# prophesier/diff-svc

Hardware: NVIDIA B200
Metric: audio-sec/s (1/RTF), 1000-step DDPM @44.1kHz + NSF-HiFiGAN (higher is better)
Workload: dtype f32 (fp16 hi/lo split x3 on tcgen05, fp32 accumulate)

## Files before the change

diffsvc_b200/csrc/diffnet.cu:

```cuda
#include "common.cuh"
#include "epilogues.cuh"
#include "simt_gemm.cuh"
#include "tc_pair.cuh"
#include "tc_splitk.cuh"
#include "tc_layer.cuh"
#include "tc_step.cuh"

#include <cmath>
#include <memory>

namespace dsvc {


__global__ void transpose_kernel(const float* __restrict__ in, float* __restrict__ out, Plane pl, int R, int Cc) {
  __shared__ float tile[32][33];
  const int b = blockIdx.z;
  const int c0 = blockIdx.x * 32, r0 = blockIdx.y * 32;
  const float* ib = in + (size_t)b * R * Cc;
  for (int i = threadIdx.y; i < 32; i += blockDim.y) {
    const int r = r0 + i, c = c0 + threadIdx.x;
    tile[i][threadIdx.x] = (r < R && c < Cc) ? ib[(size_t)r * Cc + c] : 0.f;
  }
  __syncthreads();
  for (int i = threadIdx.y; i < 32; i += blockDim.y) {
// ... 114 lines not shown
  int passes = 3;
  DevBuf w_in, b_in, w_dil, w_cond, b_cond, w_out, b_out, w_skip, b_skip, w_head, b_head;
  DevBuf dtab;
  F16Pair h_in, h_skip, h_head;
  std::vector<std::unique_ptr<F16Pair>> h_dil, h_out;
  DevBuf c_recip, c_recipm1, c_coef1, c_coef2, c_logvar, c_acp;
  bool have_schedule = false;
  int B = 0, Tmax = 0;
  int uB = 0, uT = 0;
  DevBuf rowmap;
  bool packed = false;
  bool prepared = false;
  DevBuf X, S, XS, hist, CP, cond_cl, lengths, state;
  PlaneBuf Y, Z, SP, R, XIN;
  PlaneBuf Y2;
  bool pingpong = false;
  int fused_usable = 0;
  TcMaps maps;
  DevBuf tile_tab;
  int tile_slots = 0, tile_live = 0;
  DevBuf step_flags;
  int step_bn = 0;
  int step_pairs = 0;
  DevBuf sk_slab;
  int num_sms = 148;
  cudaGraphExec_t g_ddpm = nullptr, g_plms = nullptr;
  cudaGraphExec_t g_ddpm_x = nullptr;
  uint64_t g_ddpm_x_nodes = 0;
  cudaStream_t cap_stream = nullptr;
  uint64_t g_ddpm_nodes = 0, g_plms_nodes = 0;
// ... 84 lines not shown
  DSVC_TRY(w0.upload(w->mlp0_w, (size_t)4 * C * C * 4, s));
  DSVC_TRY(b0.upload(w->mlp0_b, (size_t)4 * C * 4, s));
  DSVC_TRY(w2.upload(w->mlp2_w, (size_t)4 * C * C * 4, s));
  DSVC_TRY(b2.upload(w->mlp2_b, (size_t)C * 4, s));
  DSVC_TRY(upload_f(wp, wpv, s));
  DSVC_TRY(upload_f(bp, bpv, s));
  DSVC_TRY(t1.reserve((size_t)Tn * 4 * C * 4));
  DSVC_TRY(t2.reserve((size_t)Tn * C * 4));
  DSVC_TRY(h->dtab.reserve((size_t)Tn * L * C * 4));
  DSVC_TRY(gemm_affine(basis.as<float>(), w0.as<float>(), b0.as<float>(), t1.as<float>(), Tn, C, 4 * C, EpiAffine::ACT_MISH, s));
  DSVC_TRY(gemm_affine(t1.as<float>(), w2.as<float>(), b2.as<float>(), t2.as<float>(), Tn, 4 * C, C, EpiAffine::ACT_NONE, s));
  DSVC_TRY(gemm_affine(t2.as<float>(), wp.as<float>(), bp.as<float>(), h->dtab.as<float>(), Tn, C, L * C, EpiAffine::ACT_NONE, s));
  DSVC_CUDA(cudaStreamSynchronize(s));
  return DSVC_OK;
}

static int tc_build_maps(dsvc_diffnet* h) {
  const int M = h->cfg.mel_bins, C = h->cfg.residual_channels, L = h->cfg.residual_layers;
  const int B = h->B, T = h->Tmax;
  auto gemm = [&](TcGemmMaps& g, const PlaneBuf& a, int K, const F16Pair& w, int rows) -> int {
    DSVC_TRY(tc_make_a_map(&g.a_hi, a.hi.as<__half>(), B, T, K));
    DSVC_TRY(tc_make_a_map(&g.a_lo, a.lo.as<__half>(), B, T, K));
    DSVC_TRY(tc_make_b_map(&g.b_hi, w.hi.as<__half>(), rows, K, 128));
    DSVC_TRY(tc_make_b_map(&g.b_lo, w.lo.as<__half>(), rows, K, 128));
    DSVC_TRY(tc_make_b_map(&g.b32_hi, w.hi.as<__half>(), rows, K, 32));
    DSVC_TRY(tc_make_b_map(&g.b32_lo, w.lo.as<__half>(), rows, K, 32));
    DSVC_TRY(tc_make_b_map(&g.b64_hi, w.hi.as<__half>(), rows, K, 64));
    DSVC_TRY(tc_make_b_map(&g.b64_lo, w.lo.as<__half>(), rows, K, 64));
    return DSVC_OK;
  };
  DSVC_TRY(gemm(h->maps.in, h->XIN, M, h->h_in, C));
  DSVC_TRY(gemm(h->maps.skip, h->SP, C, h->h_skip, C));
  DSVC_TRY(gemm(h->maps.head, h->R, C, h->h_head, M));
  h->maps.dil.resize(L);
  h->maps.out.resize(L);
  for (int l = 0; l < L; ++l) {
    const PlaneBuf& yin = (h->pingpong && (l & 1)) ? h->Y2 : h->Y;
    DSVC_TRY(gemm(h->maps.dil[l], yin, C, *h->h_dil[l], 3 * 2 * C));
    DSVC_TRY(gemm(h->maps.out[l], h->Z, C, *h->h_out[l], 2 * C));
  }
  return DSVC_OK;
}

struct HeadArgs {
  int mode = HEAD_EVAL;
  float* out = nullptr;
  int tsel = 0;
};

static ConvGemmParams base_params(const float* A, const float* W, int B, int T, int Cin, int Cout, int taps, int dil) {
  ConvGemmParams p{};
  p.A = A; p.W = W; p.B = B; p.Lin = T; p.Cin = Cin; p.Cout = Cout; p.taps = taps; p.rows = T;
  p.in_stride = 1; p.in_off = (taps == 3) ? -dil : 0; p.tap_step = dil; p.nphase = 1; p.tpad = 0; p.in_slope = 1.0f;
  p.a_batch_stride = (long long)T * Cin;
// ... 6 lines not shown
  if (ctas128 >= 2 * 148) return launch_conv_gemm_tile<128, 128, 8, 8, Epi>(p, e, s);
  return launch_conv_gemm_tile<64, 128, 4, 8, Epi>(p, e, s);
}

static EpiInProj::Params mk_inproj(const dsvc_diffnet* h, int tsel) {
  EpiInProj::Params e{};
  e.bias = h->b_in.as<float>(); e.dtab = h->dtab.as<float>(); e.st = h->state.as<StepState>(); e.lengths = h->lengths.as<int>();
  e.X = h->X.as<float>(); e.Y = h->Y.view(h->tc); e.Tmax = h->Tmax; e.C = h->cfg.residual_channels; e.L = h->cfg.residual_layers;
  e.tsel = tsel; e.wscale = h->tc ? h->h_in.inv_scale : 1.f;
  e.rowmap = h->packed ? h->rowmap.as<int2>() : nullptr;
  return e;
}
static EpiGate::Params mk_gate(const dsvc_diffnet* h, int l) {
  const int C = h->cfg.residual_channels;
  EpiGate::Params e{};
  e.CP = h->CP.as<float>() + (size_t)l * h->B * h->Tmax * 2 * C; e.Z = h->Z.view(h->tc); e.Tmax = h->Tmax; e.C = C;
  e.fast = h->tc ? 1 : 0; e.wscale = h->tc ? h->h_dil[l]->inv_scale : 1.f;
  return e;
}
static EpiOutProj::Params mk_outproj(const dsvc_diffnet* h, int l, int tsel) {
  const int C = h->cfg.residual_channels;
  EpiOutProj::Params e{};
  e.bias = h->b_out.as<float>() + (size_t)l * 2 * C; e.dtab = h->dtab.as<float>(); e.st = h->state.as<StepState>();
  e.lengths = h->lengths.as<int>(); e.X = h->X.as<float>(); e.S = h->S.as<float>(); e.SP = h->SP.view(h->tc);
  e.Y = ((h->pingpong && ((l + 1) & 1)) ? h->Y2 : h->Y).view(h->tc);
  e.Tmax = h->Tmax; e.C = C; e.L = h->cfg.residual_layers; e.layer = l; e.tsel = tsel; e.fast = h->tc ? 1 : 0;
  e.wscale = h->tc ? h->h_out[l]->inv_scale : 1.f;
  e.rowmap = h->packed ? h->rowmap.as<int2>() : nullptr;
  return e;
}
static EpiSkipProj::Params mk_skip(const dsvc_diffnet* h) {
// ... 2 lines not shown
  e.wscale = h->tc ? h->h_skip.inv_scale : 1.f;
  return e;
}
static EpiHead::Params mk_head(const dsvc_diffnet* h, const HeadArgs& ha) {
  EpiHead::Params e{};
  e.bias = h->b_head.as<float>(); e.st = h->state.as<StepState>(); e.mode = ha.mode; e.B = h->B; e.Tmax = h->Tmax;
  e.M = h->cfg.mel_bins; e.out = ha.out; e.xs = h->XS.as<float>(); e.XIN = h->XIN.view(h->tc);
  e.c_recip = h->c_recip.as<float>(); e.c_recipm1 = h->c_recipm1.as<float>(); e.c_coef1 = h->c_coef1.as<float>();
  e.c_coef2 = h->c_coef2.as<float>(); e.c_logvar = h->c_logvar.as<float>();
  e.alphas_cumprod = h->c_acp.as<float>(); e.hist = h->hist.as<float>();
  e.wscale = h->tc ? h->h_head.inv_scale : 1.f;
  e.rowmap = h->packed ? h->rowmap.as<int2>() : nullptr; e.uB = h->uB; e.uT = h->uT;
  return e;
}

static int enqueue_layer_conv(dsvc_diffnet* h, int l, cudaStream_t s) {
  const int C = h->cfg.residual_channels, B = h->B, T = h->Tmax;
  const int dil = 1 << (l % h->cfg.dilation_cycle_length);
  const EpiGate::Params e = mk_gate(h, l);
  if (h->tc) {
    const TcGemmMaps& m = h->maps.dil[l];
    const char* skv = getenv("DSVC_SPLITK");
    const bool sk_wanted = (skv && atoi(skv) >= 1) || !tc_pair_enabled();
    if (h->passes == 3 && sk_wanted && h->tile_slots == 0 && h->sk_slab.bytes >= tc_splitk_slab_bytes(B, T, 2 * C) &&
        tc_splitk_eligible(B, T, 2 * C, 3, h->num_sms))
      return tc_splitk_launch<EpiGate>(m, e, h->sk_slab.as<float>(), B, T, C, 2 * C, dil, s);
    return tc_launch<EpiGate>(m, e, B, T, C, 2 * C, 3, dil, h->passes, s, tiles_of(h));
  }
  const float* W = h->w_dil.as<float>() + (size_t)l * 3 * 2 * C * C;
  return launch_fp32<EpiGate>(h, base_params(h->Y.f32.as<float>(), W, B, T, C, 2 * C, 3, dil), e, s);
}

static int enqueue_layer_out(dsvc_diffnet* h, int l, int tsel, cudaStream_t s) {
  const int C = h->cfg.residual_channels, B = h->B, T = h->Tmax;
  const EpiOutProj::Params e = mk_outproj(h, l, tsel);
  if (h->tc) return tc_launch<EpiOutProj>(h->maps.out[l], e, B, T, C, 2 * C, 1, 0, h->passes, s, tiles_of(h));
  const float* W = h->w_out.as<float>() + (size_t)l * 2 * C * C;
  return launch_fp32<EpiOutProj>(h, base_params(h->Z.f32.as<float>(), W, B, T, C, 2 * C, 1, 0), e, s);
}

static int enqueue_layer_fused(dsvc_diffnet* h, int l, int tsel, cudaStream_t s) {
  const int dil = 1 << (l % h->cfg.dilation_cycle_length);
  const TcGemmMaps* next = l + 1 < h->cfg.residual_layers ? &h->maps.dil[l + 1] : nullptr;
  return tc_layer_launch(h->maps.dil[l], h->maps.out[l], next, mk_gate(h, l), mk_outproj(h, l, tsel), h->B, h->Tmax,
                         h->cfg.residual_channels, dil, h->passes, s);
}

static bool fused_layers(const dsvc_diffnet* h) {
  if (h->tile_slots > 0) return false;
  if (!(h->tc && h->pingpong && h->fused_usable >= 1 &&
        tc_layer_shape_ok(h->B, h->Tmax, h->cfg.residual_channels))) return false;
  return tc_layer_env() >= 2 || (long long)ceil_div(h->Tmax, TC_BM) * h->B <= h->fused_usable;
}
// ... 57 lines not shown
  const char* sb = getenv("DSVC_STEP_BN");
  const int want = sb ? atoi(sb) : 0;
  if (want != 128 && M % 64 == 0 && C % 64 == 0 && cap64 > 0 && (n_ft * (2 * C / 64) <= cap64 || want == 64)) {
    const int S = n_ft * (2 * C / 64), R = ceil_div(S, cap64);
    h->step_pairs = ceil_div(S, R);
    return 64;
  }
  if (M % 128 == 0 && C % 128 == 0 && cap128 > 0) {
    const int S = n_ft * (2 * C / 128), R = ceil_div(S, cap128);
    h->step_pairs = ceil_div(S, R);
    return 128;
  }
  return 0;
}

static int enqueue_eval(dsvc_diffnet* h, const HeadArgs& ha, cudaStream_t s) {
  const int M = h->cfg.mel_bins, C = h->cfg.residual_channels, L = h->cfg.residual_layers;
  const int B = h->B, T = h->Tmax;
  if (h->step_bn > 0) return enqueue_eval_step(h, ha, s);
  {
    const EpiInProj::Params e = mk_inproj(h, ha.tsel);
    if (h->tc) DSVC_TRY(tc_launch<EpiInProj>(h->maps.in, e, B, T, M, C, 1, 0, h->passes, s, tiles_of(h)));
    else DSVC_TRY(launch_fp32<EpiInProj>(h, base_params(h->XIN.f32.as<float>(), h->w_in.as<float>(), B, T, M, C, 1, 0), e, s));
  }
  for (int l = 0; l < L; ++l) {
    if (fused_layers(h)) {
      DSVC_TRY(enqueue_layer_fused(h, l, ha.tsel, s));
      continue;
    }
    DSVC_TRY(enqueue_layer_conv(h, l, s));
    DSVC_TRY(enqueue_layer_out(h, l, ha.tsel, s));
  }
  {
    const EpiSkipProj::Params e = mk_skip(h);
    if (h->tc) DSVC_TRY(tc_launch<EpiSkipProj>(h->maps.skip, e, B, T, C, C, 1, 0, h->passes, s, tiles_of(h)));
    else DSVC_TRY(launch_fp32<EpiSkipProj>(h, base_params(h->SP.f32.as<float>(), h->w_skip.as<float>(), B, T, C, C, 1, 0), e, s));
  }
  {
    const EpiHead::Params e = mk_head(h, ha);
    if (h->tc) DSVC_TRY(tc_launch<EpiHead>(h->maps.head, e, B, T, C, M, 1, 0, h->passes, s, tiles_of(h)));
    else DSVC_TRY(launch_fp32<EpiHead>(h, base_params(h->R.f32.as<float>(), h->w_head.as<float>(), B, T, C, M, 1, 0), e, s));
  }
  return DSVC_OK;
}

static int load_x(dsvc_diffnet* h, const float* spec, cudaStream_t s) {
  const int M = h->cfg.mel_bins;
// ... 153 lines not shown
  }
  const bool ragged = tc && (int)tab.size() < dense;
  const bool ragged_changed = ragged != (h->tile_slots > 0);
  if (ragged) {
    h->tile_live = (int)tab.size();
    h->tile_slots = 2 * ceil_div(dense, 2);
    tab.resize(h->tile_slots, make_int2(0, -1));
    DSVC_TRY(h->tile_tab.reserve(tab.size() * sizeof(int2)));
    DSVC_CUDA(cudaMemcpyAsync(h->tile_tab.p, tab.data(), tab.size() * sizeof(int2), cudaMemcpyHostToDevice, s));
    DSVC_CUDA(cudaMemsetAsync(h->Y.hi.p, 0, n * C * sizeof(__half), s));
    DSVC_CUDA(cudaMemsetAsync(h->Y.lo.p, 0, n * C * sizeof(__half), s));
  } else {
    h->tile_slots = h->tile_live = 0;
  }
  DSVC_CUDA(cudaStreamSynchronize(s));
  if (resized || !h->prepared || ragged_changed) {
    h->g_ddpm_valid = h->g_plms_valid = false;
    if (tc) DSVC_TRY(tc_build_maps(h));
  }
  {
    const int bn = step_pick_bn(h);
    if (bn != h->step_bn) h->g_ddpm_valid = h->g_plms_valid = false;
    h->step_bn = bn;
    if (bn > 0) {
      const size_t fb = ((size_t)2 * ceil_div(Tmax, 2 * TC_BM) * 32 + 32) * sizeof(unsigned);
      DSVC_TRY(h->step_flags.reserve(fb));
      DSVC_CUDA(cudaMemsetAsync(h->step_flags.p, 0, fb, s));
    }
  }
  {
    Plane none{nullptr, nullptr, nullptr};
    dim3 grid(ceil_div(Tmax, 32), ceil_div(H, 32), B), block(32, 8);
    if (pack) pack_rows_kernel<<<grid, block, 0, s>>>(cond, h->cond_cl.as<float>(), none, h->rowmap.as<int2>(), Tmax, H, user_T);
    else
    transpose_kernel<<<grid, block, 0, s>>>(cond, h->cond_cl.as<float>(), none, H, Tmax);
    DSVC_LAUNCH_CHECK();
    ConvGemmParams p = base_params(h->cond_cl.as<float>(), h->w_cond.as<float>(), B, Tmax, H, L * 2 * C, 1, 0);
    EpiCondProj::Params e{};
    e.bias = h->b_cond.as<float>(); e.CP = h->CP.as<float>(); e.B = B; e.Tmax = Tmax; e.C2 = 2 * C;
    DSVC_TRY((launch_conv_gemm_tile<128, 128, 8, 8, EpiCondProj>(p, e, s)));
  }
  h->prepared = true;
  return DSVC_OK;
// ... 17 lines not shown
  DSVC_REQUIRE(hubert && mel2ph && f0 && pitch_embed && decoder_inp && f0_denorm, "dsvc_cond_encode: null argument");
  DSVC_REQUIRE(B > 0 && Th > 0 && T > 0 && H > 0 && f0_bin > 2, "dsvc_cond_encode: bad dimensions");
  DSVC_TRY(require_device());
  const float mel_min = (float)(1127.0 * std::log(1.0 + (double)f0_min / 700.0));
  const float mel_max = (float)(1127.0 * std::log(1.0 + (double)f0_max / 700.0));
  cond_encode_kernel<<<dim3(T, B), 128, 0, (cudaStream_t)stream>>>(hubert, reinterpret_cast<const long long*>(mel2ph), f0,
                                                                 pitch_embed, Th, T, H, f0_bin, mel_min, mel_max,
                                                                 decoder_inp, f0_denorm);
  DSVC_LAUNCH_CHECK();
  return DSVC_OK;
}

int dsvc_diffnet_run_layer(dsvc_diffnet_t* h, int32_t layer, int32_t part, int32_t iters, void* stream) {
  DSVC_REQUIRE(h, "dsvc_diffnet_run_layer: null handle");
  if (!h->prepared) { set_error("dsvc_diffnet_run_layer: call dsvc_diffnet_prepare first"); return DSVC_ESTATE; }
  DSVC_REQUIRE(layer >= 0 && layer < h->cfg.residual_layers && part >= 0 && part <= 3 && iters >= 0, "bad layer/part/iters");
  if (part == 3) {
    if (h->step_bn == 0) { set_error("dsvc_diffnet_run_layer: part 3 needs the step kernel (tc_step.cuh) for this shape"); return DSVC_ESTATE; }
    cudaStream_t s3 = (cudaStream_t)stream;
    set_state_kernel<<<1, 1, 0, s3>>>(h->state.as<StepState>(), 500, 1, 1ull, nullptr);
    DSVC_LAUNCH_CHECK();
    HeadArgs ha3; ha3.mode = HEAD_DDPM;
    for (int i = 0; i < iters; ++i) DSVC_TRY(enqueue_eval(h, ha3, s3));
#ifdef DSVC_TIMELINE
    {
      static long long tl[160][2 * STEP_MAXL + 3][10];
      DSVC_CUDA(cudaStreamSynchronize(s3));
      DSVC_CUDA(cudaMemcpyFromSymbol(tl, g_step_tl, sizeof(tl)));
      const int np = 2 * h->cfg.residual_layers + 3;
      const int nct = 2 * h->step_pairs;
      printf("step kernel timeline (last launch), cycles.  per phase of CTA c: start->deps | deps->first operands | first->MMAs issued | "
// ... 14 lines not shown
        double a[8] = {0, 0, 0, 0, 0, 0, 0, 0}; int n = 0;
        for (int c = 0; c < nct && c < 160; c += 2)
          for (int ph = 1 + par; ph < np - 2; ph += 2) {
            const long long* t = tl[c][ph];
            a[0] += t[1] - t[0]; a[1] += t[2] - t[1]; a[2] += t[3] - t[2]; a[3] += t[4] - t[3]; a[4] += t[5] - t[4]; a[5] += t[6] - t[5];
            a[6] += t[7] - t[6]; a[7] += tl[c][ph + 1][0] - t[0]; ++n;
          }
        printf("  mean %s: deps %.0f | first operands %.0f | MMA issue %.0f | acc ready %.0f | staged %.0f | epi %.0f | signal %.0f | total %.0f\n",
               par ? "out-proj" : "conv    ", a[0] / n, a[1] / n, a[2] / n, a[3] / n, a[4] / n, a[5] / n, a[6] / n, a[7] / n);
      }
      fflush(stdout);
    }
#endif
    return DSVC_OK;
  }
  if (part == 2 && !fused_layers(h)) {
    set_error("dsvc_diffnet_run_layer: part 2 (fused layer kernel) needs DSVC_FUSED_LAYER and a tensor-core handle whose "
              "2C/64 channel tiles form a schedulable cluster");
    return DSVC_ESTATE;
  }
  cudaStream_t s = (cudaStream_t)stream;
  set_state_kernel<<<1, 1, 0, s>>>(h->state.as<StepState>(), 0, 1, 0ull, nullptr);
  DSVC_LAUNCH_CHECK();
  for (int i = 0; i < iters; ++i) {
    if (part == 0) DSVC_TRY(enqueue_layer_conv(h, layer, s));
    else if (part == 1) DSVC_TRY(enqueue_layer_out(h, layer, 0, s));
    else DSVC_TRY(enqueue_layer_fused(h, layer, 0, s));
  }
#ifdef DSVC_TIMELINE
  if (h->tc) {
    static long long host_tl[1024][16];
    DSVC_CUDA(cudaStreamSynchronize(s));
    DSVC_CUDA(cudaMemcpyFromSymbol(host_tl, g_timeline, sizeof(host_tl)));
    const int nct = 2 * ceil_div(ceil_div(h->Tmax, TC_BM), 2) * ceil_div(2 * h->cfg.residual_channels, 64) * h->B;
    if (part == 2) {
      printf("timeline fused layer (cycles since CTA entry): setup | A:first-operands | A:mma-issued | A:epi-prefetch | A:acc-ready | "
             "A:staged | A:epi-done | fences | cluster-barrier | B:first-operands | B:mma-issued | B:epi-prefetch | B:acc-ready | "
             "B:staged | B:epi-done\n");
      for (int c = 0; c < nct && c < 1024; c += (nct > 12 ? nct / 12 : 1))
        printf("  cta %3d: %6lld %6lld %6lld %6lld %6lld %6lld %6lld %6lld %6lld %6lld %6lld %6lld %6lld %6lld %6lld\n", c,
// ... 93 lines not shown
```

diffsvc_b200/csrc/tc_gemm.cuh:

```cuda
#pragma once
#include <cuda.h>
#include <stdlib.h>
#include <cmath>

#include "common.cuh"
#include "epilogues.cuh"

namespace dsvc {

struct TcGemmMaps {
  CUtensorMap a_hi, a_lo;
  CUtensorMap b_hi, b_lo;
  CUtensorMap b32_hi, b32_lo;
  CUtensorMap b64_hi, b64_lo;
};
struct TcMaps {
  TcGemmMaps in, skip, head;
  std::vector<TcGemmMaps> dil, out;
};

struct TcTiles {
  const int2* tab = nullptr;
  int slots = 0, live = 0;
};
// ... 188 lines not shown
  asm volatile("tcgen05.ld.sync.aligned.32x32b.x4.b32 {%0, %1, %2, %3}, [%4];"
               : "=r"(u[0]), "=r"(u[1]), "=r"(u[2]), "=r"(u[3]) : "r"(taddr) : "memory");
  asm volatile("tcgen05.wait::ld.sync.aligned;" ::: "memory");
}
template <int CW> __device__ __forceinline__ void tmem_ld_cols(uint32_t taddr, float (&r)[CW]);
template <> __device__ __forceinline__ void tmem_ld_cols<8>(uint32_t taddr, float (&r)[8]) { tmem_ld8(taddr, r); }
template <> __device__ __forceinline__ void tmem_ld_cols<4>(uint32_t taddr, float (&r)[4]) { tmem_ld4(taddr, r); }
template <> __device__ __forceinline__ void tmem_ld_cols<32>(uint32_t taddr, float (&r)[32]) { tmem_ld32(taddr, r); }
template <> __device__ __forceinline__ void tmem_ld_cols<16>(uint32_t taddr, float (&r)[16]) { tmem_ld16(taddr, r); }

#ifdef DSVC_TIMELINE
__device__ long long g_timeline[1024][16];
#define TL_MARK(slot) do { if (lane == 0) g_timeline[((blockIdx.z * gridDim.y + blockIdx.y) * gridDim.x + blockIdx.x) & 1023][slot] = clock64() - tl0; } while (0)
#define TL_ENTRY() do { if (threadIdx.x == 0) { unsigned long long gt_; asm volatile("mov.u64 %0, %%globaltimer;" : "=l"(gt_)); \
  g_timeline[((blockIdx.z * gridDim.y + blockIdx.y) * gridDim.x + blockIdx.x) & 1023][15] = (long long)gt_; } } while (0)
#else
#define TL_MARK(slot) do { } while (0)
#define TL_ENTRY() do { } while (0)
#endif

template <class Epi, int BN, bool LEAN = false>
__device__ __forceinline__ void tc_epilogue(const typename Epi::Params& ep, uint8_t* smem_raw, uint32_t smem_base,
                                            uint32_t tmem_base, uint32_t tmem_full_bar, uint32_t tmem_parity, int T, int N,
                                            int m0, int ny, int b, int warp, int lane, bool two_acc
#ifdef DSVC_TIMELINE
                                            , long long tl0, int tl_off = 0
#endif
                                            , int pair_h = 0
                                            , uint32_t acc_free_bar = 0
) {
#ifndef DSVC_TIMELINE
    constexpr int tl_off = 0;
    (void)tl_off;
// ... 421 lines not shown
```

diffsvc_b200/csrc/tc_pair.cuh:

```cuda
#pragma once
#include "tc_gemm.cuh"

namespace dsvc {

template <int BN> struct TcPairCfg {
  static constexpr int H = BN / 2;
  static constexpr int P_TILE = BN * TC_BK * 2;
  static constexpr int STAGE = 2 * TC_A_TILE + P_TILE;
  static constexpr int STAGES = (BN == 64) ? 5 : (BN == 128 ? 4 : 3);
  static constexpr int SMEM = STAGES * STAGE + 1024  + 256 ;
  static_assert(4 * 32 * (BN + 4) * 4 <= STAGES * STAGE, "epilogue staging must fit in the operand ring");
};

__device__ __forceinline__ uint32_t mapa_cluster(uint32_t local_addr, uint32_t cta_rank) {
  uint32_t r;
  asm volatile("mapa.shared::cluster.u32 %0, %1, %2;" : "=r"(r) : "r"(local_addr), "r"(cta_rank));
  return r;
}
__device__ __forceinline__ void tma2_load_2d(const CUtensorMap* map, uint32_t bar, uint32_t dst, int c0, int c1) {
  asm volatile(
      "cp.async.bulk.tensor.2d.cta_group::2.shared::cluster.global.mbarrier::complete_tx::bytes [%0], [%1, {%3, %4}], [%2];"
      ::"r"(dst), "l"(map), "r"(bar), "r"(c0), "r"(c1) : "memory");
}
__device__ __forceinline__ void tma2_load_3d(const CUtensorMap* map, uint32_t bar, uint32_t dst, int c0, int c1, int c2) {
// ... 1 lines not shown
      "cp.async.bulk.tensor.3d.cta_group::2.shared::cluster.global.mbarrier::complete_tx::bytes [%0], [%1, {%3, %4, %5}], [%2];"
      ::"r"(dst), "l"(map), "r"(bar), "r"(c0), "r"(c1), "r"(c2) : "memory");
}
__device__ __forceinline__ void umma2_f16(uint32_t tmem_d, uint64_t adesc, uint64_t bdesc, uint32_t idesc, uint32_t accumulate) {
  asm volatile(
      "{\n\t.reg .pred p;\n\tsetp.ne.b32 p, %4, 0;\n\t"
      "tcgen05.mma.cta_group::2.kind::f16 [%0], %1, %2, %3, p;\n\t}"
      ::"r"(tmem_d), "l"(adesc), "l"(bdesc), "r"(idesc), "r"(accumulate) : "memory");
}
__device__ __forceinline__ void umma2_commit_both(uint32_t bar) {
  asm volatile("tcgen05.commit.cta_group::2.mbarrier::arrive::one.shared::cluster.multicast::cluster.b64 [%0], %1;"
               ::"r"(bar), "h"((uint16_t)3) : "memory");
}

template <class Epi, int BN>
__global__ void __launch_bounds__(TC_THREADS, 1)
tc_pair_kernel(const __grid_constant__ CUtensorMap tmAh, const __grid_constant__ CUtensorMap tmAl,
               const __grid_constant__ CUtensorMap tmBh, const __grid_constant__ CUtensorMap tmBl,
               const typename Epi::Params ep, int T, int K, int N, int taps, int dil, const int2* __restrict__ tiles) {
#if defined(__CUDA_ARCH__) && (__CUDA_ARCH__ >= 1000)
  using Cfg = TcPairCfg<BN>;
  constexpr int STAGES = Cfg::STAGES;
  constexpr int H = Cfg::H;
  pdl_launch_dependents();
  int m0 = blockIdx.x * TC_BM, b = blockIdx.z;
  if (tiles != nullptr) {
    const int2 t = __ldg(tiles + blockIdx.x), tp = __ldg(tiles + (blockIdx.x ^ 1u));
    if (t.y < 0 && tp.y < 0) return;
    b = t.y < 0 ? tp.x : t.x;
    m0 = t.y < 0 ? ((T + TC_BM - 1) / TC_BM) * TC_BM : t.y;
  }
  extern __shared__ uint8_t smem_raw[];
  const uint32_t smem_base = (smem_u32(smem_raw) + 1023u) & ~1023u;
  const uint32_t bar_base = smem_base + STAGES * Cfg::STAGE;
  auto full_bar = [&](int s) { return bar_base + 8u * s; };
// ... 33 lines not shown
  tc_fence_before();
  __syncthreads();
  cluster_sync_all();
  tc_fence_after();
  uint32_t tmem_base;
  asm volatile("ld.shared.u32 %0, [%1];" : "=r"(tmem_base) : "r"(tmem_slot) : "memory");
  if (warp == 3) TL_MARK(0);

  auto full_bar_leader = [&](int s) { return mapa_cluster(full_bar(s), 0u); };

  auto load_p = [&](int it, int s) {
    const int tap = it / kblocks, kb = it - tap * kblocks;
    if constexpr (BN == 256) {
      int r0, r1;
      if constexpr (Epi::kPair) {
        const int sb = tap * N + (int)blockIdx.y * 256;
        r0 = sb + (rank == 0 ? 0 : 64); r1 = r0 + 128;
      } else {
        r0 = tap * N + (int)blockIdx.y * 256 + (int)rank * 128; r1 = r0 + 64;
      }
      const uint32_t bar = full_bar_leader(s);
      const uint32_t p = tile_p(s);
      tma2_load_2d(&tmBh, bar, p, kb * TC_BK, r0);
      tma2_load_2d(&tmBh, bar, p + 64u * 128u, kb * TC_BK, r1);
      tma2_load_2d(&tmBl, bar, p + 128u * 128u, kb * TC_BK, r0);
      tma2_load_2d(&tmBl, bar, p + 192u * 128u, kb * TC_BK, r1);
    } else {
    int ra, rb;
    if constexpr (Epi::kPair) {
      const int per = 128 / BN;
      ra = tap * N + (int)(blockIdx.y / per) * 128 + (int)(blockIdx.y % per) * H;
      rb = ra + 64;
    } else {
      ra = tap * N + (int)blockIdx.y * BN;
      rb = ra + H;
    }
    const uint32_t bar = full_bar_leader(s);
    const uint32_t p = tile_p(s);
    tma2_load_2d(&tmBh, bar, p, kb * TC_BK, rank == 0 ? ra : rb);
    tma2_load_2d(&tmBl, bar, p + (uint32_t)H * 128u, kb * TC_BK, rank == 0 ? rb : ra);
    }
  };
  auto load_a = [&](int it, int s) {
    const int tap = it / kblocks, kb = it - tap * kblocks;
    const int frame = m0 + (tap - (taps >> 1)) * dil;
    const uint32_t bar = full_bar_leader(s);
    tma2_load_3d(&tmAh, bar, tile_a(s, 0), kb * TC_BK, frame, b);
    tma2_load_3d(&tmAl, bar, tile_a(s, 1), kb * TC_BK, frame, b);
  };

  if (warp == 0) {
    constexpr uint32_t tx_pair = 2u * Cfg::STAGE;
    const int pre = total < STAGES ? total : STAGES;
    if (elect_one_sync()) {
      for (int it = 0; it < pre; ++it) {
        if (rank == 0) mbar_expect_tx(full_bar(it), tx_pair);
        load_p(it, it);
      }
    }
    __syncwarp();
    pdl_wait();
    if (elect_one_sync()) {
      for (int it = 0; it < pre; ++it) load_a(it, it);
    }
    __syncwarp();
    for (int it = pre; it < total; ++it) {
      const int s = it % STAGES;
      const uint32_t ph = (uint32_t)(it / STAGES) & 1u;
      mbar_wait(empty_bar(s), ph ^ 1u);
      if (elect_one_sync()) {
        if (rank == 0) mbar_expect_tx(full_bar(s), tx_pair);
        load_a(it, s);
        load_p(it, s);
      }
      __syncwarp();
    }
// ... 20 lines not shown
            umma2_f16(tmem_base, al + koff, pd + koff, idesc_lo, 1u);
          } else {
            umma2_f16(tmem_base, ah + koff, pd + koff, idesc_hi, acc);
            umma2_f16(tmem_base, al + koff, pd + koff, idesc_lo, 1u);
          }
        }
        umma2_commit_both(empty_bar(s));
        if (it == total - 1) umma2_commit_both(tmem_full_bar);
      }
      __syncwarp();
    }
    TL_MARK(2);
  }
  pdl_wait();
#ifdef DSVC_TIMELINE
  tc_epilogue<Epi, BN>(ep, smem_raw, smem_base, tmem_base, tmem_full_bar, 0u, T, N, m0, (int)blockIdx.y, b, warp, lane, true, tl0, 0, BN == 256 ? 0 : H);
#else
  tc_epilogue<Epi, BN>(ep, smem_raw, smem_base, tmem_base, tmem_full_bar, 0u, T, N, m0, (int)blockIdx.y, b, warp, lane, true, BN == 256 ? 0 : H);
#endif
  if (warp == 4) TL_MARK(6);
  tc_fence_before();
  __syncthreads();
  cluster_sync_all();
  if (warp == 2) {
    tc_fence_after();
    asm volatile("tcgen05.dealloc.cta_group::2.sync.aligned.b32 %0, %1;" ::"r"(tmem_base), "n"(2 * BN) : "memory");
  }
#endif
}

inline bool tc_pair_enabled() {
  const char* e = getenv("DSVC_TC_PAIR");
  return !(e && atoi(e) == 0);
}

template <class Epi, int BN>
int tc_pair_launch_bn(const TcGemmMaps& m, const typename Epi::Params& e, int B, int T, int K, int N, int taps, int dil,
                      cudaStream_t s, TcTiles tt = TcTiles{}) {
  DSVC_TRY((ensure_dyn_smem<tc_pair_kernel<Epi, BN>>(TcPairCfg<BN>::SMEM)));
  cudaLaunchConfig_t cfg{};
  cfg.gridDim = tt.tab ? dim3(tt.slots, N / BN, 1) : dim3(2 * ceil_div(ceil_div(T, TC_BM), 2), N / BN, B);
  cfg.blockDim = dim3(TC_THREADS);
  cfg.dynamicSmemBytes = TcPairCfg<BN>::SMEM;
  cfg.stream = s;
  cudaLaunchAttribute attr[2];
  attr[0].id = cudaLaunchAttributeClusterDimension;
  attr[0].val.clusterDim.x = 2;
  attr[0].val.clusterDim.y = 1;
  attr[0].val.clusterDim.z = 1;
  attr[1].id = cudaLaunchAttributeProgrammaticStreamSerialization;
  attr[1].val.programmaticStreamSerializationAllowed = 1;
  cfg.attrs = attr;
  cfg.numAttrs = 2;
  const CUtensorMap& bh = (BN == 64) ? m.b32_hi : m.b64_hi;
  const CUtensorMap& bl = (BN == 64) ? m.b32_lo : m.b64_lo;
  DSVC_CUDA(cudaLaunchKernelEx(&cfg, tc_pair_kernel<Epi, BN>, m.a_hi, m.a_lo, bh, bl, e, T, K, N, taps, dil, tt.tab));
  DSVC_LAUNCH_CHECK();
  return DSVC_OK;
}

template <class Epi>
int tc_launch(const TcGemmMaps& m, const typename Epi::Params& e, int B, int T, int K, int N, int taps, int dil, int passes,
              cudaStream_t s, TcTiles tt = TcTiles{}) {
  DSVC_REQUIRE(K % TC_BK == 0, "tc_launch: K=%d must be a multiple of %d", K, TC_BK);
  if (passes == 3 && tc_pair_enabled()) {
    const int bn = tc_pick_bn(B, T, N, tt.live);
    if (bn == 64 && N % 64 == 0) return tc_pair_launch_bn<Epi, 64>(m, e, B, T, K, N, taps, dil, s, tt);
    if (bn == 128 && N % 128 == 0) return tc_pair_launch_bn<Epi, 128>(m, e, B, T, K, N, taps, dil, s, tt);
    if (bn == 256 && N % 256 == 0) return tc_pair_launch_bn<Epi, 256>(m, e, B, T, K, N, taps, dil, s, tt);
  }
  return tc_launch_single<Epi>(m, e, B, T, K, N, taps, dil, passes, s, tt);
// ... 4 lines not shown
```

Baseline: 29.87.

## Defer skip-half of out-projection into next layer's dilated-conv launch

Splits each layer's out-projection GEMM into a residual half (launched immediately) and a skip half, then runs that skip half as extra CTAs inside the next layer's dilated-conv kernel through a new two-role tc_pair2 kernel. Z is double-buffered (Z2) so the deferred skip CTAs still read the previous layer's gate output. The goal is to fill idle SMs when the grid is small and to take the skip accumulation off the critical path between layers. It is enabled only when the combined CTA count fits on the SMs. It adds a Z2 buffer, one extra launch for the last layer, and timeline instrumentation.

```diff
diff --git a/diffsvc_b200/csrc/diffnet.cu b/diffsvc_b200/csrc/diffnet.cu
--- a/diffsvc_b200/csrc/diffnet.cu
+++ b/diffsvc_b200/csrc/diffnet.cu
@@ -6,6 +6,8 @@
 #include "tc_layer.cuh"
 #include "tc_step.cuh"
 
+#include <algorithm>
+#include <climits>
 #include <cmath>
 #include <memory>
 
@@ -152,6 +154,8 @@
   DevBuf X, S, XS, hist, CP, cond_cl, lengths, state;
   PlaneBuf Y, Z, SP, R, XIN;
   PlaneBuf Y2;
+  PlaneBuf Z2;
+  bool skip_defer = false;
   bool pingpong = false;
   int fused_usable = 0;
   TcMaps maps;
@@ -266,6 +270,8 @@
   DSVC_CUDA(cudaStreamSynchronize(s));
   return DSVC_OK;
 }
+
+static const PlaneBuf& zplane(const dsvc_diffnet* h, int l) { return (h->skip_defer && (l & 1)) ? h->Z2 : h->Z; }
 
 static int tc_build_maps(dsvc_diffnet* h) {
   const int M = h->cfg.mel_bins, C = h->cfg.residual_channels, L = h->cfg.residual_layers;
@@ -289,7 +295,7 @@
   for (int l = 0; l < L; ++l) {
     const PlaneBuf& yin = (h->pingpong && (l & 1)) ? h->Y2 : h->Y;
     DSVC_TRY(gemm(h->maps.dil[l], yin, C, *h->h_dil[l], 3 * 2 * C));
-    DSVC_TRY(gemm(h->maps.out[l], h->Z, C, *h->h_out[l], 2 * C));
+    DSVC_TRY(gemm(h->maps.out[l], zplane(h, l), C, *h->h_out[l], 2 * C));
   }
   return DSVC_OK;
 }
@@ -326,7 +332,7 @@
 static EpiGate::Params mk_gate(const dsvc_diffnet* h, int l) {
   const int C = h->cfg.residual_channels;
   EpiGate::Params e{};
-  e.CP = h->CP.as<float>() + (size_t)l * h->B * h->Tmax * 2 * C; e.Z = h->Z.view(h->tc); e.Tmax = h->Tmax; e.C = C;
+  e.CP = h->CP.as<float>() + (size_t)l * h->B * h->Tmax * 2 * C; e.Z = zplane(h, l).view(h->tc); e.Tmax = h->Tmax; e.C = C;
   e.fast = h->tc ? 1 : 0; e.wscale = h->tc ? h->h_dil[l]->inv_scale : 1.f;
   return e;
 }
@@ -359,12 +365,22 @@
   return e;
 }
 
-static int enqueue_layer_conv(dsvc_diffnet* h, int l, cudaStream_t s) {
+static int enqueue_inproj(dsvc_diffnet* h, int tsel, cudaStream_t s) {
+  const int M = h->cfg.mel_bins, C = h->cfg.residual_channels;
+  const EpiInProj::Params e = mk_inproj(h, tsel);
+  if (h->tc) return tc_launch<EpiInProj>(h->maps.in, e, h->B, h->Tmax, M, C, 1, 0, h->passes, s, tiles_of(h));
+  return launch_fp32<EpiInProj>(h, base_params(h->XIN.f32.as<float>(), h->w_in.as<float>(), h->B, h->Tmax, M, C, 1, 0), e, s);
+}
+
+static int enqueue_layer_conv(dsvc_diffnet* h, int l, int tsel, cudaStream_t s) {
   const int C = h->cfg.residual_channels, B = h->B, T = h->Tmax;
   const int dil = 1 << (l % h->cfg.dilation_cycle_length);
   const EpiGate::Params e = mk_gate(h, l);
   if (h->tc) {
     const TcGemmMaps& m = h->maps.dil[l];
+    if (h->skip_defer && l > 0)
+      return tc_pair2_launch_bn<EpiGate, EpiOutProj, 64>(m, e, C, 2 * C, 3, dil, 2 * C / 64, h->maps.out[l - 1],
+                                                          mk_outproj(h, l - 1, tsel), C, 2 * C, 1, 0, C / 64, C / 64, B, T, s);
     const char* skv = getenv("DSVC_SPLITK");
     const bool sk_wanted = (skv && atoi(skv) >= 1) || !tc_pair_enabled();
     if (h->passes == 3 && sk_wanted && h->tile_slots == 0 && h->sk_slab.bytes >= tc_splitk_slab_bytes(B, T, 2 * C) &&
@@ -379,9 +395,16 @@
 static int enqueue_layer_out(dsvc_diffnet* h, int l, int tsel, cudaStream_t s) {
   const int C = h->cfg.residual_channels, B = h->B, T = h->Tmax;
   const EpiOutProj::Params e = mk_outproj(h, l, tsel);
+  if (h->skip_defer) return tc_pair_launch_bn<EpiOutProj, 64>(h->maps.out[l], e, B, T, C, 2 * C, 1, 0, s, TcTiles{}, 0, C / 64);
   if (h->tc) return tc_launch<EpiOutProj>(h->maps.out[l], e, B, T, C, 2 * C, 1, 0, h->passes, s, tiles_of(h));
   const float* W = h->w_out.as<float>() + (size_t)l * 2 * C * C;
   return launch_fp32<EpiOutProj>(h, base_params(h->Z.f32.as<float>(), W, B, T, C, 2 * C, 1, 0), e, s);
+}
+
+static int enqueue_layer_skip(dsvc_diffnet* h, int l, int tsel, cudaStream_t s) {
+  const int C = h->cfg.residual_channels;
+  return tc_pair_launch_bn<EpiOutProj, 64>(h->maps.out[l], mk_outproj(h, l, tsel), h->B, h->Tmax, C, 2 * C, 1, 0, s, TcTiles{},
+                                          C / 64, C / 64);
 }
 
 static int enqueue_layer_fused(dsvc_diffnet* h, int l, int tsel, cudaStream_t s) {
@@ -469,23 +492,32 @@
   return 0;
 }
 
+static bool skip_defer_pick(const dsvc_diffnet* h) {
+  const char* e = getenv("DSVC_SKIP_DEFER");
+  if (e && atoi(e) == 0) return false;
+  const char* skv = getenv("DSVC_SPLITK");
+  if (skv && atoi(skv) >= 1) return false;
+  const int C = h->cfg.residual_channels;
+  if (!(h->tc && h->passes == 3 && tc_pair_enabled()) || h->tile_slots > 0 || h->step_bn > 0 || fused_layers(h)) return false;
+  if (C % 64 != 0 || tc_pick_bn(h->B, h->Tmax, 2 * C) != 64) return false;
+  const long long ft = (long long)tc_pair_frame_ctas(h->Tmax) * h->B;
+  return ft * (2 * C / 64) + ft * (C / 64) <= h->num_sms;
+}
+
 static int enqueue_eval(dsvc_diffnet* h, const HeadArgs& ha, cudaStream_t s) {
   const int M = h->cfg.mel_bins, C = h->cfg.residual_channels, L = h->cfg.residual_layers;
   const int B = h->B, T = h->Tmax;
   if (h->step_bn > 0) return enqueue_eval_step(h, ha, s);
-  {
-    const EpiInProj::Params e = mk_inproj(h, ha.tsel);
-    if (h->tc) DSVC_TRY(tc_launch<EpiInProj>(h->maps.in, e, B, T, M, C, 1, 0, h->passes, s, tiles_of(h)));
-    else DSVC_TRY(launch_fp32<EpiInProj>(h, base_params(h->XIN.f32.as<float>(), h->w_in.as<float>(), B, T, M, C, 1, 0), e, s));
-  }
+  DSVC_TRY(enqueue_inproj(h, ha.tsel, s));
   for (int l = 0; l < L; ++l) {
     if (fused_layers(h)) {
       DSVC_TRY(enqueue_layer_fused(h, l, ha.tsel, s));
       continue;
     }
-    DSVC_TRY(enqueue_layer_conv(h, l, s));
-    DSVC_TRY(enqueue_layer_out(h, l, ha.tsel, s));
-  }
+    DSVC_TRY(enqueue_layer_conv(h, l, ha.tsel, s));
+    if (!h->skip_defer || l + 1 < L) DSVC_TRY(enqueue_layer_out(h, l, ha.tsel, s));
+  }
+  if (h->skip_defer) DSVC_TRY(enqueue_layer_skip(h, L - 1, ha.tsel, s));
   {
     const EpiSkipProj::Params e = mk_skip(h);
     if (h->tc) DSVC_TRY(tc_launch<EpiSkipProj>(h->maps.skip, e, B, T, C, C, 1, 0, h->passes, s, tiles_of(h)));
@@ -669,10 +701,6 @@
     h->tile_slots = h->tile_live = 0;
   }
   DSVC_CUDA(cudaStreamSynchronize(s));
-  if (resized || !h->prepared || ragged_changed) {
-    h->g_ddpm_valid = h->g_plms_valid = false;
-    if (tc) DSVC_TRY(tc_build_maps(h));
-  }
   {
     const int bn = step_pick_bn(h);
     if (bn != h->step_bn) h->g_ddpm_valid = h->g_plms_valid = false;
@@ -682,6 +710,13 @@
       DSVC_TRY(h->step_flags.reserve(fb));
       DSVC_CUDA(cudaMemsetAsync(h->step_flags.p, 0, fb, s));
     }
+  }
+  const bool defer = skip_defer_pick(h);
+  if (defer) DSVC_TRY(h->Z2.reserve(n * C, tc));
+  if (resized || !h->prepared || ragged_changed || defer != h->skip_defer) {
+    h->g_ddpm_valid = h->g_plms_valid = false;
+    h->skip_defer = defer;
+    if (tc) DSVC_TRY(tc_build_maps(h));
   }
   {
     Plane none{nullptr, nullptr, nullptr};
@@ -729,7 +764,7 @@
 int dsvc_diffnet_run_layer(dsvc_diffnet_t* h, int32_t layer, int32_t part, int32_t iters, void* stream) {
   DSVC_REQUIRE(h, "dsvc_diffnet_run_layer: null handle");
   if (!h->prepared) { set_error("dsvc_diffnet_run_layer: call dsvc_diffnet_prepare first"); return DSVC_ESTATE; }
-  DSVC_REQUIRE(layer >= 0 && layer < h->cfg.residual_layers && part >= 0 && part <= 3 && iters >= 0, "bad layer/part/iters");
+  DSVC_REQUIRE(layer >= 0 && layer < h->cfg.residual_layers && part >= 0 && part <= 4 && iters >= 0, "bad layer/part/iters");
   if (part == 3) {
     if (h->step_bn == 0) { set_error("dsvc_diffnet_run_layer: part 3 needs the step kernel (tc_step.cuh) for this shape"); return DSVC_ESTATE; }
     cudaStream_t s3 = (cudaStream_t)stream;
@@ -774,6 +809,60 @@
 #endif
     return DSVC_OK;
   }
+  if (part == 4) {
+    if (!h->tc || h->step_bn > 0 || fused_layers(h)) {
+      set_error("dsvc_diffnet_run_layer: part 4 needs the per-layer tensor-core kernels");
+      return DSVC_ESTATE;
+    }
+    cudaStream_t s4 = (cudaStream_t)stream;
+    for (int run = 0; run < 2; ++run) {
+      set_state_kernel<<<1, 1, 0, s4>>>(h->state.as<StepState>(), 500, 1, 1ull, nullptr);
+      DSVC_LAUNCH_CHECK();
+      DSVC_TRY(enqueue_inproj(h, 0, s4));
+      for (int l = 0; l <= layer; ++l) {
+        DSVC_TRY(enqueue_layer_conv(h, l, 0, s4));
+        if (l < layer || run == 1) DSVC_TRY(enqueue_layer_out(h, l, 0, s4));
+      }
+#ifdef DSVC_TIMELINE
+      static long long tl4[1024][16];
+      DSVC_CUDA(cudaStreamSynchronize(s4));
+      DSVC_CUDA(cudaMemcpyFromSymbol(tl4, g_timeline, sizeof(tl4)));
+      const int C = h->cfg.residual_channels, gx = tc_pair_frame_ctas(h->Tmax), bn = tc_pick_bn(h->B, h->Tmax, 2 * C);
+      const int n_conv = 2 * C / bn, n_skip = (h->skip_defer && layer > 0) ? C / 64 : 0;
+      const int rows = run == 0 ? n_conv + n_skip : (h->skip_defer ? C / 64 : 2 * C / bn);
+      const int nct = gx * rows * h->B;
+      if (nct > 1024) { printf("part 4: %d CTAs, more than the timeline holds\n", nct); continue; }
+      auto role = [&](int c) { const int y = (c / gx) % rows; return run == 1 ? 2 : (y < n_conv ? 0 : 1); };
+      long long e0 = tl4[0][15], rel = tl4[0][13];
+      for (int c = 0; c < nct; ++c) { e0 = std::min(e0, tl4[c][15]); rel = std::min(rel, tl4[c][13]); }
+      const char* names[3] = {"gate", "skip", "out"};
+      printf("timeline part 4, layer %d, %s kernel (%s schedule), %d CTAs; ns after the first CTA entry; release = the earliest "
+             "return from griddepcontrol.wait (%lld)\n", layer, run == 0 ? "conv" : "out-projection",
+             h->skip_defer ? "deferred-skip" : "layer-by-layer", nct, rel - e0);
+      for (int r = 0; r < 3; ++r) {
+        int n = 0, waiting = 0;
+        long long last_in = 0, first_done = LLONG_MAX, last_done = 0, last_ops = 0;
+        for (int c = 0; c < nct; ++c) {
+          if (role(c) != r) continue;
+          ++n;
+          waiting += tl4[c][13] - rel < 500;
+          last_in = std::max(last_in, tl4[c][15] - e0);
+          first_done = std::min(first_done, tl4[c][14] - e0);
+          last_done = std::max(last_done, tl4[c][14] - e0);
+          last_ops = std::max(last_ops, tl4[c][13] - e0);
+        }
+        if (n == 0) continue;
+        printf("  %-4s %3d CTAs: %3d waiting at the release (past the wait < 0.5 us after it) | last entry %6lld | last past the wait "
+               "%6lld | done %6lld .. %6lld\n", names[r], n, waiting, last_in, last_ops, first_done, last_done);
+      }
+      for (int c = 0; c < nct; c += 2)
+        printf("  cta %3d %-4s: entry %6lld | past wait %6lld | first operands +%5lld cyc | done %6lld\n", c, names[role(c)],
+               tl4[c][15] - e0, tl4[c][13] - e0, tl4[c][1], tl4[c][14] - e0);
+      fflush(stdout);
+#endif
+    }
+    return DSVC_OK;
+  }
   if (part == 2 && !fused_layers(h)) {
     set_error("dsvc_diffnet_run_layer: part 2 (fused layer kernel) needs DSVC_FUSED_LAYER and a tensor-core handle whose "
               "2C/64 channel tiles form a schedulable cluster");
@@ -783,7 +872,7 @@
   set_state_kernel<<<1, 1, 0, s>>>(h->state.as<StepState>(), 0, 1, 0ull, nullptr);
   DSVC_LAUNCH_CHECK();
   for (int i = 0; i < iters; ++i) {
-    if (part == 0) DSVC_TRY(enqueue_layer_conv(h, layer, s));
+    if (part == 0) DSVC_TRY(enqueue_layer_conv(h, layer, 0, s));
     else if (part == 1) DSVC_TRY(enqueue_layer_out(h, layer, 0, s));
     else DSVC_TRY(enqueue_layer_fused(h, layer, 0, s));
   }
diff --git a/diffsvc_b200/csrc/tc_gemm.cuh b/diffsvc_b200/csrc/tc_gemm.cuh
--- a/diffsvc_b200/csrc/tc_gemm.cuh
+++ b/diffsvc_b200/csrc/tc_gemm.cuh
@@ -226,9 +226,12 @@
 #define TL_MARK(slot) do { if (lane == 0) g_timeline[((blockIdx.z * gridDim.y + blockIdx.y) * gridDim.x + blockIdx.x) & 1023][slot] = clock64() - tl0; } while (0)
 #define TL_ENTRY() do { if (threadIdx.x == 0) { unsigned long long gt_; asm volatile("mov.u64 %0, %%globaltimer;" : "=l"(gt_)); \
   g_timeline[((blockIdx.z * gridDim.y + blockIdx.y) * gridDim.x + blockIdx.x) & 1023][15] = (long long)gt_; } } while (0)
+#define TL_GT(slot) do { if (threadIdx.x == 0) { unsigned long long gt_; asm volatile("mov.u64 %0, %%globaltimer;" : "=l"(gt_)); \
+  g_timeline[((blockIdx.z * gridDim.y + blockIdx.y) * gridDim.x + blockIdx.x) & 1023][slot] = (long long)gt_; } } while (0)
 #else
 #define TL_MARK(slot) do { } while (0)
 #define TL_ENTRY() do { } while (0)
+#define TL_GT(slot) do { } while (0)
 #endif
 
 template <class Epi, int BN, bool LEAN = false>
diff --git a/diffsvc_b200/csrc/tc_pair.cuh b/diffsvc_b200/csrc/tc_pair.cuh
--- a/diffsvc_b200/csrc/tc_pair.cuh
+++ b/diffsvc_b200/csrc/tc_pair.cuh
@@ -39,11 +39,9 @@
 }
 
 template <class Epi, int BN>
-__global__ void __launch_bounds__(TC_THREADS, 1)
-tc_pair_kernel(const __grid_constant__ CUtensorMap tmAh, const __grid_constant__ CUtensorMap tmAl,
-               const __grid_constant__ CUtensorMap tmBh, const __grid_constant__ CUtensorMap tmBl,
-               const typename Epi::Params ep, int T, int K, int N, int taps, int dil, const int2* __restrict__ tiles) {
-#if defined(__CUDA_ARCH__) && (__CUDA_ARCH__ >= 1000)
+__device__ __forceinline__ void tc_pair_cta(const CUtensorMap& tmAh, const CUtensorMap& tmAl, const CUtensorMap& tmBh,
+                                            const CUtensorMap& tmBl, const typename Epi::Params& ep, int T, int K, int N,
+                                            int taps, int dil, const int2* __restrict__ tiles, int ny) {
   using Cfg = TcPairCfg<BN>;
   constexpr int STAGES = Cfg::STAGES;
   constexpr int H = Cfg::H;
@@ -107,10 +105,10 @@
     if constexpr (BN == 256) {
       int r0, r1;
       if constexpr (Epi::kPair) {
-        const int sb = tap * N + (int)blockIdx.y * 256;
+        const int sb = tap * N + ny * 256;
         r0 = sb + (rank == 0 ? 0 : 64); r1 = r0 + 128;
       } else {
-        r0 = tap * N + (int)blockIdx.y * 256 + (int)rank * 128; r1 = r0 + 64;
+        r0 = tap * N + ny * 256 + (int)rank * 128; r1 = r0 + 64;
       }
       const uint32_t bar = full_bar_leader(s);
       const uint32_t p = tile_p(s);
@@ -122,10 +120,10 @@
     int ra, rb;
     if constexpr (Epi::kPair) {
       const int per = 128 / BN;
-      ra = tap * N + (int)(blockIdx.y / per) * 128 + (int)(blockIdx.y % per) * H;
+      ra = tap * N + (ny / per) * 128 + (ny % per) * H;
       rb = ra + 64;
     } else {
-      ra = tap * N + (int)blockIdx.y * BN;
+      ra = tap * N + ny * BN;
       rb = ra + H;
     }
     const uint32_t bar = full_bar_leader(s);
@@ -153,6 +151,7 @@
     }
     __syncwarp();
     pdl_wait();
+    TL_GT(13);
     if (elect_one_sync()) {
       for (int it = 0; it < pre; ++it) load_a(it, it);
     }
@@ -203,18 +202,42 @@
   }
   pdl_wait();
 #ifdef DSVC_TIMELINE
-  tc_epilogue<Epi, BN>(ep, smem_raw, smem_base, tmem_base, tmem_full_bar, 0u, T, N, m0, (int)blockIdx.y, b, warp, lane, true, tl0, 0, BN == 256 ? 0 : H);
+  tc_epilogue<Epi, BN>(ep, smem_raw, smem_base, tmem_base, tmem_full_bar, 0u, T, N, m0, ny, b, warp, lane, true, tl0, 0, BN == 256 ? 0 : H);
 #else
-  tc_epilogue<Epi, BN>(ep, smem_raw, smem_base, tmem_base, tmem_full_bar, 0u, T, N, m0, (int)blockIdx.y, b, warp, lane, true, BN == 256 ? 0 : H);
+  tc_epilogue<Epi, BN>(ep, smem_raw, smem_base, tmem_base, tmem_full_bar, 0u, T, N, m0, ny, b, warp, lane, true, BN == 256 ? 0 : H);
 #endif
   if (warp == 4) TL_MARK(6);
   tc_fence_before();
   __syncthreads();
+  TL_GT(14);
   cluster_sync_all();
   if (warp == 2) {
     tc_fence_after();
     asm volatile("tcgen05.dealloc.cta_group::2.sync.aligned.b32 %0, %1;" ::"r"(tmem_base), "n"(2 * BN) : "memory");
   }
+}
+
+template <class Epi, int BN>
+__global__ void __launch_bounds__(TC_THREADS, 1)
+tc_pair_kernel(const __grid_constant__ CUtensorMap tmAh, const __grid_constant__ CUtensorMap tmAl,
+               const __grid_constant__ CUtensorMap tmBh, const __grid_constant__ CUtensorMap tmBl,
+               const typename Epi::Params ep, int T, int K, int N, int taps, int dil, const int2* __restrict__ tiles, int ny0) {
+#if defined(__CUDA_ARCH__) && (__CUDA_ARCH__ >= 1000)
+  tc_pair_cta<Epi, BN>(tmAh, tmAl, tmBh, tmBl, ep, T, K, N, taps, dil, tiles, ny0 + (int)blockIdx.y);
+#endif
+}
+
+template <class EpiA, class EpiB, int BN>
+__global__ void __launch_bounds__(TC_THREADS, 1)
+tc_pair2_kernel(const __grid_constant__ CUtensorMap aAh, const __grid_constant__ CUtensorMap aAl,
+                const __grid_constant__ CUtensorMap aBh, const __grid_constant__ CUtensorMap aBl,
+                const typename EpiA::Params epA, int KA, int NA, int tapsA, int dilA, int nA,
+                const __grid_constant__ CUtensorMap bAh, const __grid_constant__ CUtensorMap bAl,
+                const __grid_constant__ CUtensorMap bBh, const __grid_constant__ CUtensorMap bBl,
+                const typename EpiB::Params epB, int KB, int NB, int tapsB, int dilB, int nyB, int T) {
+#if defined(__CUDA_ARCH__) && (__CUDA_ARCH__ >= 1000)
+  if ((int)blockIdx.y < nA) tc_pair_cta<EpiA, BN>(aAh, aAl, aBh, aBl, epA, T, KA, NA, tapsA, dilA, nullptr, (int)blockIdx.y);
+  else tc_pair_cta<EpiB, BN>(bAh, bAl, bBh, bBl, epB, T, KB, NB, tapsB, dilB, nullptr, nyB + (int)blockIdx.y - nA);
 #endif
 }
 
@@ -223,27 +246,54 @@
   return !(e && atoi(e) == 0);
 }
 
+inline int tc_pair_frame_ctas(int T) { return 2 * ceil_div(ceil_div(T, TC_BM), 2); }
+
+struct TcPairLaunch {
+  cudaLaunchConfig_t cfg{};
+  cudaLaunchAttribute attr[2];
+  TcPairLaunch(dim3 grid, int smem, cudaStream_t s) {
+    cfg.gridDim = grid;
+    cfg.blockDim = dim3(TC_THREADS);
+    cfg.dynamicSmemBytes = smem;
+    cfg.stream = s;
+    attr[0].id = cudaLaunchAttributeClusterDimension;
+    attr[0].val.clusterDim.x = 2;
+    attr[0].val.clusterDim.y = 1;
+    attr[0].val.clusterDim.z = 1;
+    attr[1].id = cudaLaunchAttributeProgrammaticStreamSerialization;
+    attr[1].val.programmaticStreamSerializationAllowed = 1;
+    cfg.attrs = attr;
+    cfg.numAttrs = 2;
+  }
+};
+
+template <int BN> const CUtensorMap& tc_pair_bh(const TcGemmMaps& m) { return BN == 64 ? m.b32_hi : m.b64_hi; }
+template <int BN> const CUtensorMap& tc_pair_bl(const TcGemmMaps& m) { return BN == 64 ? m.b32_lo : m.b64_lo; }
+
 template <class Epi, int BN>
 int tc_pair_launch_bn(const TcGemmMaps& m, const typename Epi::Params& e, int B, int T, int K, int N, int taps, int dil,
-                      cudaStream_t s, TcTiles tt = TcTiles{}) {
+                      cudaStream_t s, TcTiles tt = TcTiles{}, int ny0 = 0, int n_ny = 0) {
   DSVC_TRY((ensure_dyn_smem<tc_pair_kernel<Epi, BN>>(TcPairCfg<BN>::SMEM)));
-  cudaLaunchConfig_t cfg{};
-  cfg.gridDim = tt.tab ? dim3(tt.slots, N / BN, 1) : dim3(2 * ceil_div(ceil_div(T, TC_BM), 2), N / BN, B);
-  cfg.blockDim = dim3(TC_THREADS);
-  cfg.dynamicSmemBytes = TcPairCfg<BN>::SMEM;
-  cfg.stream = s;
-  cudaLaunchAttribute attr[2];
-  attr[0].id = cudaLaunchAttributeClusterDimension;
-  attr[0].val.clusterDim.x = 2;
-  attr[0].val.clusterDim.y = 1;
-  attr[0].val.clusterDim.z = 1;
-  attr[1].id = cudaLaunchAttributeProgrammaticStreamSerialization;
-  attr[1].val.programmaticStreamSerializationAllowed = 1;
-  cfg.attrs = attr;
-  cfg.numAttrs = 2;
-  const CUtensorMap& bh = (BN == 64) ? m.b32_hi : m.b64_hi;
-  const CUtensorMap& bl = (BN == 64) ? m.b32_lo : m.b64_lo;
-  DSVC_CUDA(cudaLaunchKernelEx(&cfg, tc_pair_kernel<Epi, BN>, m.a_hi, m.a_lo, bh, bl, e, T, K, N, taps, dil, tt.tab));
+  const int ny = n_ny > 0 ? n_ny : N / BN;
+  DSVC_REQUIRE(ny0 >= 0 && ny0 + ny <= N / BN, "tc_pair_launch: channel tiles %d..%d of %d", ny0, ny0 + ny - 1, N / BN);
+  TcPairLaunch l(tt.tab ? dim3(tt.slots, ny, 1) : dim3(tc_pair_frame_ctas(T), ny, B), TcPairCfg<BN>::SMEM, s);
+  DSVC_CUDA(cudaLaunchKernelEx(&l.cfg, tc_pair_kernel<Epi, BN>, m.a_hi, m.a_lo, tc_pair_bh<BN>(m), tc_pair_bl<BN>(m), e, T, K, N,
+                               taps, dil, tt.tab, ny0));
+  DSVC_LAUNCH_CHECK();
+  return DSVC_OK;
+}
+
+template <class EpiA, class EpiB, int BN>
+int tc_pair2_launch_bn(const TcGemmMaps& mA, const typename EpiA::Params& eA, int KA, int NA, int tapsA, int dilA, int nA,
+                       const TcGemmMaps& mB, const typename EpiB::Params& eB, int KB, int NB, int tapsB, int dilB, int nyB, int nB,
+                       int B, int T, cudaStream_t s) {
+  DSVC_TRY((ensure_dyn_smem<tc_pair2_kernel<EpiA, EpiB, BN>>(TcPairCfg<BN>::SMEM)));
+  DSVC_REQUIRE(KA % TC_BK == 0 && KB % TC_BK == 0 && nA > 0 && nA <= NA / BN && nB > 0 && nyB >= 0 && nyB + nB <= NB / BN,
+               "tc_pair2_launch: bad roles (K %d / %d, tiles %d of %d, %d..%d of %d)", KA, KB, nA, NA / BN, nyB, nyB + nB - 1, NB / BN);
+  TcPairLaunch l(dim3(tc_pair_frame_ctas(T), nA + nB, B), TcPairCfg<BN>::SMEM, s);
+  DSVC_CUDA(cudaLaunchKernelEx(&l.cfg, tc_pair2_kernel<EpiA, EpiB, BN>, mA.a_hi, mA.a_lo, tc_pair_bh<BN>(mA), tc_pair_bl<BN>(mA), eA,
+                               KA, NA, tapsA, dilA, nA, mB.a_hi, mB.a_lo, tc_pair_bh<BN>(mB), tc_pair_bl<BN>(mB), eB, KB, NB,
+                               tapsB, dilB, nyB, T));
   DSVC_LAUNCH_CHECK();
   return DSVC_OK;
 }
```

Result: faster. 31.27, median of 6 (+4.7%).
